# DataCTE/SDXL-Training-Improvements

Measured on AMD Instinct MI355X. Metric: images/sec/node SDXL-base 1024^2 bf16 fwd+bwd, higher is better.
Workload: dtype bf16; 1 GPU; method=ddpm v_prediction + zero_terminal_snr + MinSNR(5), SDXL-base UNet fwd+bwd, batch 4/GPU, 1024^2 (latent 128x128); global_batch=4, parallelism=dp1, weights=synthetic (counter-hash init of the 2,567,463,684-parameter SDXL-base UNet)

## Files before the change

### sdxl-training-improvements_amd/csrc/engine.hip

```cpp
#include "engine.h"

#include <stdarg.h>
#include <stdlib.h>

#ifdef SDXL_DIAG
int g_knobs[SDXL_NKNOBS] = {0};
#endif
static thread_local char g_err[1024] = "";
void sdxl_set_error(const char* fmt, ...) {
  va_list ap;
  va_start(ap, fmt);
  vsnprintf(g_err, sizeof(g_err), fmt, ap);
  va_end(ap);
}
const char* sdxl_get_error() { return g_err; }

#define CHK(x)            \
  do {                    \
    int _r = (x);         \
    if (_r) return _r;    \
  } while (0)

static inline size_t align_up(size_t v, size_t a) { return (v + a - 1) / a * a; }

// ... 44 lines not shown
    if (hipEventCreateWithFlags(&e, hipEventDisableTiming | hipEventDisableSystemFence) != hipSuccess) return nullptr;
    ev_pool.push_back(e);
  }
  return ev_pool[ev_used++];
}
template <class F>
static int on_side(Plan& p, hipStream_t main, F&& fn) {
  Engine& e = *p.eng;
  if (!e.use_side || !e.side || gemm_profiling()) return fn(main);
  hipEvent_t ev = e.next_event();
  if (!ev) { sdxl_set_error("hipEventCreate failed"); return 2; }
  HIP_CHECK_RET(hipEventRecord(ev, main));
  HIP_CHECK_RET(hipStreamWaitEvent(e.side, ev, 0));
  e.side_dirty = true;
  if (!e.side_leaves.empty()) {
    std::vector<std::function<int(hipStream_t)>> v;
    v.swap(e.side_leaves);
    for (auto& leaf : v) CHK(leaf(e.side));
  }
  return fn(e.side);
}
template <class F>
static int side_leaf(Plan& p, hipStream_t main, F&& fn) {
  Engine& e = *p.eng;
  if (!e.use_side || !e.side || gemm_profiling() || KNOB(2) == 16) return on_side(p, main, fn);
  e.side_leaves.emplace_back(std::function<int(hipStream_t)>(fn));
  return 0;
}
static int launch_wgrad_bucket(Plan& p, hipStream_t main, std::vector<GemmP>& v) {
  if (v.empty()) return 0;
  GemmP g = v[0];
  if (v.size() > 1) {
    g.splitk = 1;
    gemm_fill_group(g, v.data(), (int)v.size());
  }
  v.clear();
  if (g.splitk > 1) g.anyorder = 0;
  return on_side(p, main, [&g](hipStream_t s2) -> int { return launch_gemm(g, s2); });
}
int Engine::defer_wgrad(Plan& p, hipStream_t main, const GemmP& g, int grp) {
  for (auto& b : wg_pending) {
    if (b.empty() || (b[0].M == g.M && b[0].N == g.N && b[0].K == g.K && b[0].accumulate == g.accumulate)) {
      b.push_back(g);
      if ((int)b.size() >= grp) return launch_wgrad_bucket(p, main, b);
      return 0;
    }
  }
  wg_pending.emplace_back(1, g);
  if (grp <= 1) return launch_wgrad_bucket(p, main, wg_pending.back());
  return 0;
}
int Engine::flush_wgrads(Plan& p, hipStream_t main) {
  if (!side_leaves.empty()) CHK(on_side(p, main, [](hipStream_t) -> int { return 0; }));
  for (auto& b : wg_pending) CHK(launch_wgrad_bucket(p, main, b));
  return 0;
}
int Engine::flush_ln_params(Plan& p, hipStream_t main) {
  size_t i = 0;
  while (i < ln_pending.size()) {
    LnRedBatch b;
    b.n = 0;
    while (i < ln_pending.size() && b.n < LN_RED_MAX) b.e[b.n++] = ln_pending[i++];
    CHK(on_side(p, main, [&b](hipStream_t s2) -> int { return launch_ln_param_reduce(b, s2); }));
  }
  ln_pending.clear();
  return 0;
// ... 97 lines not shown
  size_t dy32_off = NONE;
  size_t dy_off = NONE;
  Plan::GradDst dx, dres;
  int ggroup = 64;
  Act* gact = nullptr;
  Act* gu = nullptr;
  LinearOp(Act* x_, Act* y_, PRef w_, PRef b_, int K_, int N_, Act* resid_) : x(x_), y(y_), resid(resid_), w(w_), b(b_), K(K_), N(N_) {}
  void describe(const Plan&, sdxl_plan_op_desc* d) const override {
    d->kind = SDXL_OP_LINEAR;
    desc_tensor(d, 0, x); desc_tensor(d, 1, y); desc_tensor(d, 2, resid); desc_tensor(d, 3, gact); desc_tensor(d, 4, gu);
    desc_param(d, w, b);
    d->K = K; d->N = N; d->splitk = splitk; d->wgroup = wgroup; d->crcfg = crcfg; d->crsplit = crsplit; d->fsplit = fsplit; d->dsplit = dsplit;
    d->delta_on = delta_on ? 1 : 0; d->ln_mode = ln_mode; d->ggroup = ggroup; d->resid_alias = resid_alias;
    d->dy_off = dy_off; d->dy32_off = dy32_off; d->dx_out = dx.out; d->dx_addend = dx.addend; d->dres_out = dres.out; d->dres_addend = dres.addend;
    if (ln_mode == 1) desc_lost(d, INTACT_GRAD, 0);
  }
  int fwd(Plan& p, hipStream_t st) override {
    GemmP g = linear_fwd_problem(p.P(x), x->ld(), p.eng->Wp(w), p.P(y), y->ld(), (int)x->rows, N, K, b.off == NONE ? nullptr : p.eng->Wp(b),
                                 resid ? p.P(resid) : nullptr, resid ? resid->ld() : 0);
    if (gact) gemm_attach_geglu_fwd(g, ggroup, p.P(gact), gact->ld());
    if (fsplit > 1 && !hoist_fwd) { g.splitk = fsplit; g.slab = p.F(p.slab_main_off); }
    return launch_gemm(g, st);
  }
  void plan_bwd(Plan& p) override {
    dy_off = y->goff;
    if (resid) {
      resid_alias = p.grad_alias(resid, y) ? 1 : 0;
      if (!resid_alias) dres = p.grad_dst(resid);
    }
    if (gu) dx = p.grad_dst(gu);
    else if (x->need_grad) dx = p.grad_dst(x);
    splitk = linear_wgrad_splitk(N, K, x->rows);
    wgroup = gemm_pick_group(N, K, 1, x->rows, splitk);
    want_slab(p, N, K, 1, splitk);
    crcfg = cr256_wgrad_cfg(N, K, x->rows, b.off != NONE);
    if (crcfg) { crsplit = cr256_pick_splitk(N, K, x->rows, crcfg); want_slab(p, N, K, 1, crsplit); }
    if (!gact) { fsplit = gemm_pick_splitk_small((int)x->rows, N, K, 3); want_slab_main(p, (int)x->rows, N, fsplit); }
    if (const Engine::LoraOpSel* lo = p.eng->lora_op(w)) {
      const size_t tu = lora_grad_tu_elems((int)lo->host.size(), p.eng->lora.rank, (int)x->rows);
      const size_t pf = (size_t)lora_grad_chunks((int)x->rows) * lo->part_unit;
      if (tu > p.lg_tu_elems) p.lg_tu_elems = tu;
      if (pf > p.lg_part_floats) p.lg_part_floats = pf;
    }
    if (delta_attn && !(!gu && x->need_grad)) attn_set_delta_fused(delta_attn, false);
    if (!gu && x->need_grad) {
      dsplit = gemm_pick_splitk_small((int)x->rows, K, N, 2);
      if (KNOB(3) > 1 && N >= (KNOB(4) > 0 ? KNOB(4) : 8192) && N % (64 * KNOB(3)) == 0 && dsplit == 1) dsplit = KNOB(3);
      want_slab_main(p, (int)x->rows, K, dsplit);
      if (delta_attn) {
        delta_on = attn_delta_wanted(delta_attn) && dsplit <= 1 && K % 128 == 0;
        attn_set_delta_fused(delta_attn, delta_on);
      }
      if (SDXL_LN_EPILOGUE && ln_src && KNOB(26) != 0 && dsplit == 1 && dx.addend == NONE && !x->parent && gemm_ln_cfg((int)x->rows, K, N) &&
          ln_fuse_plan(ln_src, p, KNOB(26) == 2 ? 2 : 1))
        ln_mode = KNOB(26) == 2 ? 2 : 1;
    }
  }
  int bwd(Plan& p, hipStream_t st, bool first) override {
    const bf16* dy = p.GP(dy_off);
    const int M = (int)x->rows;
    if (dy32_off != NONE) {
      auto& cs = p.eng->cs_pending;
      for (size_t i = 0; i < cs.size();) {
        LnRedBatch rb;
        rb.n = 0;
        while (i < cs.size() && rb.n < LN_RED_MAX) rb.e[rb.n++] = cs[i++];
// ... 1088 lines not shown
```

### sdxl-training-improvements_amd/csrc/gemm.hip

```cpp
#include "gemm_tiles.h"

#include <stdio.h>
#include <stdlib.h>

#include <type_traits>
#include <vector>

#define BM 128
#ifndef GEMM_DIRECT_EPILOGUE
#define GEMM_DIRECT_EPILOGUE 1
#endif

static int g_mode256 = 1;
static int g_force_cfg = 0;
#ifdef SDXL_DIAG
static int g_sk_mode = 0;
#endif

static constexpr int cdiv_c(int a, int b) { return (a + b - 1) / b; }
__device__ unsigned g_ln_spin_error = 0;
__device__ __forceinline__ float row16_sum(float v) {
  v += __builtin_bit_cast(float, __builtin_amdgcn_update_dpp(0, __builtin_bit_cast(int, v), 0x111, 0xf, 0xf, true));
  v += __builtin_bit_cast(float, __builtin_amdgcn_update_dpp(0, __builtin_bit_cast(int, v), 0x112, 0xf, 0xf, true));
  v += __builtin_bit_cast(float, __builtin_amdgcn_update_dpp(0, __builtin_bit_cast(int, v), 0x114, 0xf, 0xf, true));
// ... 972 lines not shown
          for (int e = 0; e < 8; ++e) {
            oa[e] = (bf16)xa[e];
            ot[e] = (bf16)xt[e];
            og[e] = (bf16)((float)oa[e] * gelu_f((float)ot[e]));
          }
          *(bf16x8*)((bf16*)p.C + (long)m * p.ldc + na) = oa;
          *(bf16x8*)((bf16*)p.C + (long)m * p.ldc + nt) = ot;
          *(bf16x8*)(p.aux + (long)m * p.ldaux + (n0 >> 1) + col) = og;
        } else {
          const int n = n0 + col;
          if (n >= p.N) continue;
          const int Gp = p.geglu_group;
          const long cu = (long)(n / Gp) * (2 * Gp) + (n % Gp);
          bf16x8 ua = *(const bf16x8*)(p.aux + (long)m * p.ldaux + cu);
          bf16x8 ut = *(const bf16x8*)(p.aux + (long)m * p.ldaux + cu + Gp);
          bf16x8 oa, ot;
#pragma unroll
          for (int e = 0; e < 8; ++e) {
            const float dv = (float)(bf16)Cs[row * LDC + col + e], tv = (float)ut[e];
            float cdf, pdf;
            gelu_cdf_pdf(tv, &cdf, &pdf);
            oa[e] = (bf16)(dv * tv * cdf);
            ot[e] = (bf16)(dv * (float)ua[e] * fmaf(tv, pdf, cdf));
          }
          *(bf16x8*)((bf16*)p.C + (long)m * p.ldc + cu) = oa;
          *(bf16x8*)((bf16*)p.C + (long)m * p.ldc + cu + Gp) = ot;
        }
      }
    }
    __syncthreads();
  }
}

__global__ void splitk_reduce_kernel(const float* __restrict__ slab, float* __restrict__ C, int M, int cols, long ldc,
                                     long slab_ld, int splitk, int accumulate, bf16* __restrict__ Cb, float cb_scale,
                                     float* __restrict__ bias_grad) {
  const int vpr = cols / 4;
  for (long i = (long)blockIdx.x * blockDim.x + threadIdx.x; i < (long)M * vpr; i += (long)gridDim.x * blockDim.x) {
    long m = i / vpr;
    int c = (int)(i - m * vpr) * 4;
    if (bias_grad && c == 0) {
      const float* tail = slab + (long)splitk * M * slab_ld + m;
      float b = 0.f;
      for (int s = 0; s < splitk; ++s) b += tail[(long)s * M];
      bias_grad[m] += b;
    }
    f32x4 a = accumulate ? *(const f32x4*)(C + m * ldc + c) : (f32x4){0.f, 0.f, 0.f, 0.f};
    for (int s = 0; s < splitk; ++s) {
      f32x4 v = *(const f32x4*)(slab + ((long)s * M + m) * slab_ld + c);
      a[0] += v[0]; a[1] += v[1]; a[2] += v[2]; a[3] += v[3];
    }
    if (Cb) {
      bf16x4 o;
      o[0] = (bf16)(a[0] * cb_scale); o[1] = (bf16)(a[1] * cb_scale); o[2] = (bf16)(a[2] * cb_scale); o[3] = (bf16)(a[3] * cb_scale);
      *(bf16x4*)(Cb + m * ldc + c) = o;
    } else {
      *(f32x4*)(C + m * ldc + c) = a;
    }
  }
}

__global__ void splitk_epilogue_kernel(const float* __restrict__ slab, bf16* __restrict__ C, int M, int N, long ldc, long slab_ld,
                                       int splitk, const bf16* __restrict__ bias, const bf16* __restrict__ resid, long ldr,
                                       const bf16* __restrict__ rowvec, long ldv, int rows_per_batch) {
  const int vpr = N / 8;
  for (long i = (long)blockIdx.x * blockDim.x + threadIdx.x; i < (long)M * vpr; i += (long)gridDim.x * blockDim.x) {
    const long m = i / vpr;
    const int n = (int)(i - m * vpr) * 8;
    float x[8] = {0.f, 0.f, 0.f, 0.f, 0.f, 0.f, 0.f, 0.f};
    for (int s = 0; s < splitk; ++s) {
      const float* sp = slab + ((long)s * M + m) * slab_ld + n;
      const f32x4 a = *(const f32x4*)sp, b = *(const f32x4*)(sp + 4);
      x[0] += a[0]; x[1] += a[1]; x[2] += a[2]; x[3] += a[3]; x[4] += b[0]; x[5] += b[1]; x[6] += b[2]; x[7] += b[3];
    }
    if (bias) {
      const bf16x8 v = *(const bf16x8*)(bias + n);
#pragma unroll
      for (int e = 0; e < 8; ++e) x[e] += (float)v[e];
    }
    if (rowvec) {
      const bf16x8 v = *(const bf16x8*)(rowvec + (m / rows_per_batch) * ldv + n);
#pragma unroll
      for (int e = 0; e < 8; ++e) x[e] += (float)v[e];
    }
    if (resid) {
      const bf16x8 v = *(const bf16x8*)(resid + m * ldr + n);
#pragma unroll
      for (int e = 0; e < 8; ++e) x[e] += (float)v[e];
    }
    bf16x8 o;
#pragma unroll
    for (int e = 0; e < 8; ++e) o[e] = (bf16)x[e];
// ... 368 lines not shown
    ARG_CHECK(((uintptr_t)p.rowvec & 15) == 0 && p.ldv % 8 == 0 && p.rows_per_batch >= 1,
              "gemm: the row vector must be 16-byte aligned, ldv=%ld a multiple of 8, rows_per_batch=%d at least 1", p.ldv, p.rows_per_batch);
  if (p.form == GEMM_TN) {
    ARG_CHECK(p.M % 8 == 0, "gemm TN: M=%d must be a multiple of 8", p.M);
    ARG_CHECK(p.out_f32, "gemm TN: only fp32 output is implemented");
    ARG_CHECK(p.ldc % 4 == 0, "gemm TN: ldc=%ld must be a multiple of 4", p.ldc);
  } else {
    ARG_CHECK(p.K % 8 == 0, "gemm: K=%d must be a multiple of 8", p.K);
    ARG_CHECK(!p.out_f32, "gemm NT/NN: bf16 output");
    if (p.splitk > 1 && (!gemm_fast_ok(p, 64) || p.geglu || p.N % 8 != 0)) p.splitk = 1;
    ARG_CHECK(p.ldc % 8 == 0, "gemm: ldc=%ld must be a multiple of 8", p.ldc);
    if (p.accumulate) { p.resid = (const bf16*)p.C; p.ldr = p.ldc; }
    if (p.geglu) {
      if (p.geglu_group == 0) p.geglu_group = 64;
      ARG_CHECK(p.geglu == 2 ? p.geglu_group % 8 == 0 : (p.geglu_group == 64 || p.geglu_group == 80), "gemm: geglu group %d (forward: 64 or 80)", p.geglu_group);
      const int G = p.geglu_group;
      ARG_CHECK((p.geglu == 1 && p.form == GEMM_NT && p.N % (2 * G) == 0) || (p.geglu == 2 && p.form == GEMM_NN && p.N % G == 0),
                "gemm: geglu mode %d does not fit form %d / N=%d / group %d", p.geglu, p.form, p.N, G);
      ARG_CHECK(p.aux && p.ldaux % 8 == 0 && ((uintptr_t)p.aux & 15) == 0 && p.taps == 1, "gemm: geglu needs an aligned aux matrix");
      ARG_CHECK(!p.resid && !p.rowvec && (p.geglu == 1 || !p.bias), "gemm: geglu epilogue takes no residual / row vector");
    }
  }
  if (p.form == GEMM_TN) {
    ARG_CHECK(!p.geglu, "gemm TN: no geglu epilogue");
    ARG_CHECK(!p.Cb || (((uintptr_t)p.Cb & 7) == 0), "gemm TN: bf16 destination must be 8-byte aligned");
  } else {
    ARG_CHECK(!p.Cb, "gemm: the bf16 gradient destination is a TN (wgrad) option");
  }
  if (p.splitk < 1) p.splitk = 1;
  if (p.delta_out)
    ARG_CHECK(p.form == GEMM_NN && p.splitk == 1 && p.taps == 1 && !p.geglu && p.delta_o && p.delta_nq > 0 && p.delta_heads > 0 && p.delta_ldo % 8 == 0,
              "gemm: the Delta epilogue takes a plain, unsplit NN problem (form %d, splitk %d)", p.form, p.splitk);
  if (p.group > 1) {
    ARG_CHECK(p.form == GEMM_TN && p.taps == 1 && p.splitk == 1 && p.group <= GEMM_MAX_GROUP,
              "gemm: grouped launches are TN, one tap, no split-K, at most %d problems", GEMM_MAX_GROUP);
    for (int i = 0; i < p.group; ++i)
      ARG_CHECK(p.gA[i] && p.gB[i] && p.gC[i] && (((uintptr_t)p.gA[i] | (uintptr_t)p.gB[i] | (uintptr_t)p.gC[i]) & 15) == 0,
                "gemm: grouped operands must be set and 16-byte aligned");
    p.A = p.gA[0]; p.B = p.gB[0]; p.C = p.gC[0]; p.bias_grad = p.gbias_grad[0]; p.Cb = p.gCb[0];
  } else {
    p.group = 0;
  }
  {
    p.xcd_px = 0;
    {
      const int gx = cdiv(p.N, 128), gy = cdiv(p.M, BM);
      double best = 1e30;
      for (int px = 1; px <= 8; px *= 2) {
        const int py = 8 / px;
        if (gx % px || gy % py) continue;
        double cost = (double)p.N / px + (double)p.M / py;
        if (cost < best) { best = cost; p.xcd_px = px; }
      }
    }
  }
  if (p.splitk > 1) {
    ARG_CHECK(p.slab != nullptr, "gemm: split-K needs a slab scratch buffer");
    if (p.form != GEMM_TN && p.splitk > p.K / 64 * p.taps) p.splitk = p.K / 64 * p.taps;
    p.slab_ld = p.form == GEMM_TN ? (long)p.N * p.taps : (long)p.N;
  }
  if (p.ln_x) {
    ARG_CHECK(SDXL_LN_EPILOGUE, "gemm: the LayerNorm-backward epilogue exists in the diagnostics build only");
    ARG_CHECK(p.form == GEMM_NN && p.taps == 1 && p.splitk == 1 && !p.geglu && !p.resid && !p.bias && !p.rowvec && !p.delta_out && !p.up2,
              "gemm: the LayerNorm-backward epilogue takes a plain NN problem");
    const int lc = gemm_ln_cfg(p.M, p.N, p.K);
    ARG_CHECK(lc != 0 && (p.cfg == lc || p.cfg == 0), "gemm: LayerNorm-backward epilogue: M=%d N=%d K=%d cfg=%d does not fit (gemm_ln_cfg)", p.M, p.N, p.K, p.cfg);
    p.cfg = lc;
    ARG_CHECK(p.ln_stats && p.ln_gamma && p.ln_dx && p.ln_part && p.ln_epoch > 0 && p.ln_ldx % 8 == 0 && p.ln_ldo % 8 == 0 && ((uintptr_t)p.ln_part & 15) == 0 &&
              (((uintptr_t)p.ln_x | (uintptr_t)p.ln_dx | (uintptr_t)p.ln_addend | (uintptr_t)p.ln_gamma) & 15) == 0,
              "gemm: LayerNorm-backward epilogue: missing or misaligned buffers");
  }
  return 0;
}

GemmRoute gemm_route(const GemmP& p) {
  const bool tn = p.form == GEMM_TN, split = p.splitk > 1;
  const int fc = p.cfg > 0 ? p.cfg : g_force_cfg;
  const int post = !split ? GEMM_POST_NONE : tn ? GEMM_POST_REDUCE : GEMM_POST_EPILOGUE;
  auto k128 = [&]() -> GemmRoute {
    const int c = gemm_route_cfg128(p);
    const bool fast = gemm_fast_ok(p, c == 2 ? 32 : 64);
    return {GEMM_K128, c == 23 && !fast ? 3 : c, fast, post};
  };
  if (p.ln_x) return k128();
  {
    bool use = fc == 7 || fc == 8;
    const bool pl_pf = fc == 8 || KNOB(31) == 1;
    if (!use && fc == 0 && KNOB(30) != 64 && p.taps == 1 && !tn) {
      const int bnp = p.N % 160 == 0 ? 160 : 128;
      const long tiles = (long)cdiv(p.M, BM) * cdiv(p.N, bnp);
      const int k30 = KNOB(30) ? KNOB(30) : 3;
      const bool one_round = tiles <= 256 && tiles > 128;
      use = ((k30 & 1) && p.form == GEMM_NT && one_round) || ((k30 & 2) && p.form == GEMM_NN && one_round) || ((k30 & 512) && p.form == GEMM_NN && one_round && p.K >= 2560) ||
            ((k30 & 16) && tiles > 128 && tiles % 256 == 0) || ((k30 & 1024) && p.form == GEMM_NT && tiles > 256 && tiles % 256 == 0) || (k30 & 32);
    }
    if (use && pl_applicable(p)) return {GEMM_KPL, pl_pf ? 8 : 7, false, GEMM_POST_NONE};
  }
  if (fc >= 31 && fc <= 36 && !p.delta_out && cr256_applicable(p)) {
    bool biasg = tn && p.bias_grad;
    for (int i = 0; tn && i < p.group; ++i) biasg = biasg || p.gbias_grad[i];
    return {GEMM_KCR256, fc == 31 && biasg ? 32 : fc, false, tn ? post : GEMM_POST_NONE};
  }
#ifdef SDXL_DIAG
  if (g_sk_mode && !p.delta_out && !(!tn && split) && (g_sk_mode == 2 ? gemm_sk_applicable(p) : gemm_use_sk(p))) return {GEMM_KSK, 0, false, GEMM_POST_NONE};
#endif
  if (g_mode256 && p.group <= 1 && !p.Cb && !p.delta_out && !(!tn && split) && gemm256_applicable(p)) {
    const bool geglu256 = p.geglu == 1 && p.geglu_group == 64 && (long)(p.M / 256) * (p.N / 256) >= 256;
    if (g_mode256 == 2 || gemm_use256(p.form, p.M, p.N, p.K, p.splitk) || geglu256) return {GEMM_K256, 0, false, post};
  }
  if (tn && p.taps != 1 && conv_wgrad3_applicable(p) && conv_wgrad3_policy(p.M, p.N, p.K, p.Wm, p.sm)) return {GEMM_KCONV_WGRAD3, 0, false, post};
  if (tn && p.taps == 1 && wgrad256_applicable(p) && wgrad256_policy(p.M, p.N, p.K)) return {GEMM_KWGRAD256, 0, false, post};
  return k128();
}
int gemm_route_checked(GemmP p, GemmRoute* r) {
  if (int e = gemm_check(p)) return e;
  *r = gemm_route(p);
  return 0;
}

static int launch_gemm_post(const GemmP& p, int post, hipStream_t st) {
  if (post == GEMM_POST_NONE) return 0;
  const int cols = post == GEMM_POST_REDUCE ? p.N * p.taps : p.N;
  const long nv = (long)p.M * (cols / (post == GEMM_POST_REDUCE ? 4 : 8));
  int g = (int)((nv + 255) / 256);
  if (g > 2048) g = 2048;
  if (post == GEMM_POST_REDUCE)
    hipLaunchKernelGGL(splitk_reduce_kernel, dim3(g), dim3(256), 0, st, p.slab, (float*)p.C, p.M, cols, p.ldc, p.slab_ld, p.splitk, p.accumulate, p.Cb,
                       p.cb_scale, p.up2 == 1 ? nullptr : p.bias_grad);
  else
    hipLaunchKernelGGL(splitk_epilogue_kernel, dim3(g), dim3(256), 0, st, p.slab, (bf16*)p.C, p.M, p.N, p.ldc, p.slab_ld, p.splitk,
                       p.bias, p.resid, p.ldr, p.rowvec, p.ldv, p.rows_per_batch > 0 ? p.rows_per_batch : 1);
  HIP_CHECK_RET(hipGetLastError());
  return 0;
}

static int launch_gemm_impl(const GemmP& pin, hipStream_t st) {
  GemmP p = pin;
  if (int e = gemm_check(p)) return e;
  const GemmRoute r = gemm_route(p);
  const bool conv = p.taps != 1;
  int rc;
  switch (r.kernel) {
    case GEMM_KPL: return launch_pl(p, 0, st, r.cfg == 8);
    case GEMM_KCR256: rc = launch_cr256(p, (r.cfg == 31 || r.cfg == 33 || r.cfg == 36) ? 160 : 128, st, r.cfg == 33 || r.cfg == 34, r.cfg == 35 || r.cfg == 36); break;
#ifdef SDXL_DIAG
    case GEMM_KSK: {
      GemmP q = p;
      q.splitk = 1;
      return launch_gemm_sk(&q, 1, st);
    }
#endif
    case GEMM_K256: rc = launch_gemm256(p, st); break;
    case GEMM_KCONV_WGRAD3: rc = launch_conv_wgrad3(p, st); break;
    case GEMM_KWGRAD256: rc = launch_wgrad256(p, st); break;
    default:
      if (p.form == GEMM_NT) rc = conv ? launch_one<GEMM_NT, true>(p, r, st) : launch_one<GEMM_NT, false>(p, r, st);
      else if (p.form == GEMM_TN) rc = conv ? launch_one<GEMM_TN, true>(p, r, st) : launch_one<GEMM_TN, false>(p, r, st);
      else if (p.form == GEMM_NN) rc = conv ? launch_one<GEMM_NN, true>(p, r, st) : launch_one<GEMM_NN, false>(p, r, st);
      else ARG_CHECK(false, "gemm: unknown form %d", p.form);
// ... 123 lines not shown
```

### sdxl-training-improvements_amd/csrc/hooks.hip

```cpp
#include "capi.h"

static int hook_scratch(size_t bytes, void** out) {
  static char* buf = nullptr;
  static size_t cap = 0;
  if (bytes > cap) {
    if (buf) { (void)hipFree(buf); buf = nullptr; cap = 0; }
    HIP_CHECK_RET(hipMalloc((void**)&buf, bytes));
    cap = bytes;
  }
  *out = buf;
  return 0;
}
static int hook_floats(size_t n, float** out) { return hook_scratch(n * sizeof(float), (void**)out); }
static int dense_problem(int form, const void* A, const void* B, void* C, int M, int N, int K, const void* bias, const void* resid, int accumulate,
                         GemmP* g) {
  const bf16 *a = (const bf16*)A, *b = (const bf16*)B, *r = (const bf16*)resid;
  ARG_CHECK(form == GEMM_NT || form == GEMM_NN || form == GEMM_TN, "gemm: unknown form %d", form);
  if (form == GEMM_NT) *g = linear_fwd_problem(a, K, b, C, N, M, N, K, (const bf16*)bias, r, N);
  else if (form == GEMM_NN) { *g = linear_dgrad_problem(a, K, b, C, N, M, N, K, r, N); g->bias = (const bf16*)bias; }
  else { *g = linear_wgrad_problem(a, M, b, N, (float*)C, M, N, K, (float*)bias); if (r) { g->resid = r; g->ldr = N; } }
  g->accumulate = accumulate;
  return 0;
}

// ... 180 lines not shown
  memset(out, 0, sizeof(*out));
  size_t* const offs[] = {&out->dy_off, &out->dx_out, &out->dx_addend, &out->dres_out, &out->dres_addend, &out->d3_out, &out->d3_addend, &out->dy32_off,
                          &out->w_off, &out->b_off, &out->stats_off, &out->lse_off, &out->delta_off, &out->rv32_off, &out->planar_off, &out->weff_off,
                          &out->dweff_off, &out->s2_planar_off};
  for (size_t* o : offs) *o = SDXL_PLAN_NONE;
  for (int r = 0; r < SDXL_PLAN_ROLES; ++r) plan_describe_tensor(out->t[r], nullptr);
  out->intact_after_step = ~0u;
  const Op& op = *p.ops[i];
  out->seg = op.seg; out->hoist_fwd = op.hoist_fwd ? 1 : 0;
  op.describe(p, out);
  return 0;
}
int sdxl_debug_plan_tail(sdxl_handle* h, sdxl_plan_tail* out, size_t out_bytes) {
  ARG_CHECK(out_bytes == sizeof(sdxl_plan_tail), "plan tail: the caller's struct has %zu bytes, the library's %zu", out_bytes, sizeof(sdxl_plan_tail));
  H_CHECK(h);
  ARG_CHECK(h->e.cur, "no plan: call sdxl_plan first");
  ARG_CHECK(out, "null output");
  const Plan& p = *h->e.cur;
  memset(out, 0, sizeof(*out));
  out->B = p.B; out->H = p.H; out->W = p.W; out->ctx = p.ctx;
  plan_describe_tensor(out->x_in, p.x_in); plan_describe_tensor(out->pred, p.pred); plan_describe_tensor(out->ehs, p.ehs);
  out->tp32_off = p.tp32_off; out->tp32_bytes = p.tp32_bytes; out->t_off = p.t_off; out->tid_off = p.tid_off; out->loss_off = p.loss_off;
  out->workspace_bytes = p.ws_bytes;
  return 0;
}

int sdxl_op_wgrad_group(int n, const void* const* dy, const void* const* x, float* const* dw, float* const* dbias, int Mo, int No,
                        int rows, int accumulate, void* st) {
  ARG_CHECK(n >= 1 && n <= GEMM_MAX_GROUP, "wgrad group of %d (1..%d)", n, GEMM_MAX_GROUP);
  GemmP v[GEMM_MAX_GROUP];
  for (int i = 0; i < n; ++i) v[i] = linear_wgrad_problem((const bf16*)dy[i], Mo, (const bf16*)x[i], No, dw[i], Mo, No, rows, dbias ? dbias[i] : nullptr);
  GemmP g = v[0];
  g.accumulate = accumulate;
  gemm_fill_group(g, v, n);
  return launch_gemm(g, (hipStream_t)st);
}

int sdxl_op_conv3x3_fwd(const void* x, const void* w, const void* bias, void* y, int B, int H, int W, int Cin, int Cout,
                        int stride, void* st) {
  GemmP g = conv3x3_fwd_problem(B, H, W, Cin, Cout, stride);
  g.A = (const bf16*)x; g.B = (const bf16*)w; g.C = y;
  g.bias = (const bf16*)bias;
  g.splitk = conv3x3_fwd_splitk(B, H, W, Cin, Cout, stride);
  if (g.splitk > 1) CHK(hook_floats(gemm_slab_floats(g.M, Cout, 1, g.splitk), &g.slab));
  return launch_gemm(g, (hipStream_t)st);
}
int sdxl_op_upconv3x3_fwd(const void* x, const void* w, const void* bias, void* weff, void* planar, void* y, int B, int H, int W,
                          int Cin, int Cout, void* st) {
  const int Mp = 4 * (int)upconv_plane_rows(B, H, W);
  int splitk = upconv3x3_fwd_splitk(B, H, W, Cin, Cout);
  float* slab = nullptr;
  if (splitk > 1) CHK(hook_floats(gemm_slab_floats(Mp, Cout, 1, splitk), &slab));
  return launch_upconv3x3_fwd((const bf16*)x, (const bf16*)w, (const bf16*)bias, (bf16*)weff, (bf16*)planar, (bf16*)y, B, H, W, Cin, Cout,
                              splitk, slab, (hipStream_t)st);
}
int sdxl_op_upconv3x3_dgrad(const void* dy, const void* weff, void* planar, void* dx, const void* addend, int B, int H, int W, int Cin,
                            int Cout, void* st) {
  int splitk = upconv3x3_dgrad_splitk(B, H, W, Cin, Cout);
  float* slab = nullptr;
  if (splitk > 1) CHK(hook_floats(gemm_slab_floats(B * H * W, Cin, 1, splitk), &slab));
  return launch_upconv3x3_dgrad((const bf16*)dy, (const bf16*)weff, (bf16*)planar, (bf16*)dx, (const bf16*)addend, B, H, W, Cin, Cout, splitk,
                                slab, 0, (hipStream_t)st);
}
#ifdef SDXL_DIAG
int sdxl_op_conv3x3_s2_fwd(const void* x, const void* w, const void* bias, void* xplanar, void* y, int B, int H, int W, int Cin, int Cout,
                           void* st) {
// ... 367 lines not shown
```

### sdxl-training-improvements_amd/csrc/kernels.h

```cpp
#pragma once
#include "common.h"

#define SDXL_NKNOBS 40
#ifdef SDXL_DIAG
extern int g_knobs[SDXL_NKNOBS];
#define KNOB(i) (g_knobs[(i)])
constexpr bool SDXL_DIAG_BUILD = true;
constexpr bool SDXL_UP2_3 = true;
constexpr bool SDXL_LN_EPILOGUE = true;
#else
#define KNOB(i) 0
constexpr bool SDXL_DIAG_BUILD = false;
constexpr bool SDXL_UP2_3 = false;
constexpr bool SDXL_LN_EPILOGUE = false;
#endif

enum { GEMM_NT = 0, GEMM_NN = 1, GEMM_TN = 2 };
#define GEMM_LAUNCH(kernel, grid, block, smem, st, p)                                                          \
  do {                                                                                                         \
    if ((p).anyorder) hipExtLaunchKernelGGL(kernel, grid, block, smem, st, nullptr, nullptr, hipExtAnyOrderLaunch, p); \
    else hipLaunchKernelGGL(kernel, grid, block, smem, st, p);                                                 \
  } while (0)

#define GEMM_MAX_GROUP 4
// ... 89 lines not shown
GemmP conv3x3_fwd_problem(int B, int H, int W, int Cin, int Cout, int stride);
GemmP conv3x3_dgrad_problem(int B, int H, int W, int Cin, int Cout, int stride);
GemmP conv3x3_wgrad_problem(int B, int H, int W, int Cin, int Cout, int stride);
GemmP linear_fwd_problem(const bf16* x, long ldx, const bf16* w, void* y, long ldy, int M, int N, int K, const bf16* bias, const bf16* resid, long ldr);
GemmP linear_dgrad_problem(const bf16* dy, long ldy, const bf16* w, void* dx, long ldx, int M, int N, int K, const bf16* addend, long ldr);
GemmP linear_wgrad_problem(const bf16* dy, long ldy, const bf16* x, long ldx, float* dw, int Mo, int No, int rows, float* bias_grad);
void gemm_attach_geglu_fwd(GemmP& g, int group, bf16* gact, long ldgact);
void gemm_attach_geglu_bwd(GemmP& g, int group, bf16* u, long ldu);
void gemm_attach_delta(GemmP& g, const bf16* o, long ldo, float* delta, int nq, int heads);
void gemm_attach_ln_bwd(GemmP& g, const bf16* x, long ldx, const float* stats, const bf16* gamma, bf16* dx, const bf16* addend, float* part, int epoch,
                        float* pcol);
void gemm_fill_group(GemmP& g, const GemmP* v, int n);
int launch_gemm256(const GemmP& p, hipStream_t st);
void gemm256_set_tail(bool on);
#ifdef SDXL_DIAG
bool gemm_sk_applicable(const GemmP& p);
int launch_gemm_sk(const GemmP* problems, int n, hipStream_t st);
int launch_gemm_multi(const GemmP* problems, int n, hipStream_t st);
void gemm_set_sk_mode(int mode);
int gemm_sk_mode();
bool gemm_use_sk(const GemmP& p);
void gemm_sk_set_workers(int n);
int gemm_ln_error(unsigned* out);
int gemm_sk_error(hipStream_t st, unsigned* out);
#endif
bool conv_wgrad3_applicable(const GemmP& p);
bool conv_wgrad3_policy(int M, int N, long red, int Wm, int stride);
int conv_wgrad3_pick_splitk(int M, int N, long red);
int launch_conv_wgrad3(const GemmP& p, hipStream_t st);
void conv_wgrad3_set_enabled(bool on);
bool wgrad256_applicable(const GemmP& p);
bool wgrad256_policy(int M, int N, long red);
int wgrad256_pick_splitk(int M, int N, long red);
int launch_wgrad256(const GemmP& p, hipStream_t st);
void wgrad256_set_enabled(bool on);
bool cr256_applicable(const GemmP& p);
int launch_cr256(const GemmP& p, int bn, hipStream_t st, bool deep = false, bool phased = false);
int cr256_wgrad_cfg(int M, int N, long red, bool bias);
bool pl_applicable(const GemmP& p);
int launch_pl(const GemmP& p, int bn, hipStream_t st, bool prefetch = false);
int launch_pl_prefetch_b(const GemmP& p, int parts, hipStream_t st);
int gemm_ln_cfg(int M, int N, int K);
size_t gemm_ln_part_floats(int M, int N);
size_t gemm_ln_pcol_floats(int M, int N);
int gemm_ln_rowblocks(int M);
int cr256_pick_splitk(int M, int N, long red, int cfg);
int gemm_profile_begin();
FILE* launch_log();
bool gemm_profiling();
int gemm_profile_end(double* flops, double* ms, int* launches);

struct AttnP {
  const bf16 *Q, *K, *V;
  bf16* O;
  float* LSE;
  int B, H, Nq, Nk;
  long ldq, ldk, ldv, ldo;
  const bf16* dO;
  long lddo;
  bf16 *dQ, *dK, *dV;
  long lddq, lddk, lddv;
  float* Delta;
  int accumulate;
  int qsplit;
  float* part;
  int prio;
// ... 320 lines not shown
```

### sdxl-training-improvements_amd/csrc/wgrad256.hip

```cpp
#include "gemm_tiles.h"

namespace {

constexpr int WL_BM = 256, WL_BN = 160, WL_BK = 64, WL_S = 3;
constexpr int WL_A_BYTES = WL_BK * WL_BM * 2;
constexpr int WL_B_BYTES = WL_BK * WL_BN * 2;
constexpr int WL_STAGE = WL_A_BYTES + WL_B_BYTES;
constexpr int WL_SMEM = WL_S * WL_STAGE + 1024;
constexpr int WL_NL = 7;

__global__ __launch_bounds__(512, 2) void wgrad256_kernel(const GemmP p) {
  extern __shared__ __attribute__((aligned(16))) char smem[];
  const int tid = threadIdx.x, lane = tid & 63;
  const int wave = __builtin_amdgcn_readfirstlane(tid >> 6);
  const int wm = wave >> 1, wn = wave & 1;
  const int l16 = lane & 15, g = lane >> 4;
  int bx, by, split;
  xcd_seq_map(p.xcd_bh, bx, by, split);
  const int n0 = bx * WL_BN, m0 = by * WL_BM;
  const int ktiles = p.K / WL_BK;
  const int chunk = (ktiles + p.splitk - 1) / p.splitk;
  const int kt_begin = split * chunk;
  const int kt_end = min(ktiles, kt_begin + chunk);
  const int T = kt_end - kt_begin;
  const bf16* zsrc = (const bf16*)g_zero16;
  const unsigned lds_base = lds_addr_of(smem);
  const unsigned pad_dst = lds_base + WL_S * WL_STAGE;

  const bf16* pa[4];
  long sa[4];
#pragma unroll
  for (int j = 0; j < 4; ++j) {
    const int c = wave + 8 * j;
    const int sub = c >> 4, cc = c & 15;
    const int krow = cc * 4 + (lane >> 4);
    const int m = m0 + sub * 128 + (nc_logical<128>(krow, lane & 15) << 3);
    const bool ok = m < p.M;
    pa[j] = ok ? p.A + ((long)kt_begin * WL_BK + krow) * p.lda + m : zsrc;
    sa[j] = ok ? (long)WL_BK * p.lda : 0;
  }
  const bf16* pb[3];
  long sb[3];
#pragma unroll
  for (int j = 0; j < 3; ++j) {
    const int c = wave + 8 * j;
    const int q = c * 64 + lane;
    const int krow = q / 20, pv = q - krow * 20;
    const int n = n0 + (nc_logical<160>(krow, pv) << 3);
    const bool ok = c < 20 && n < p.N;
    pb[j] = ok ? p.B + ((long)kt_begin * WL_BK + krow) * p.ldb + n : zsrc;
    sb[j] = ok ? (long)WL_BK * p.ldb : 0;
  }
  auto issue_piece = [&](int pc, int slot, bool live) {
    const unsigned At = lds_base + slot * WL_STAGE, Bt = At + WL_A_BYTES;
#pragma unroll
    for (int j = 0; j < 4; ++j)
      if (pc == j) {
        lds_dma16_global(live ? (const void*)pa[j] : (const void*)zsrc, At + (wave + 8 * j) * 1024);
        pa[j] += sa[j];
      }
#pragma unroll
    for (int j = 0; j < 3; ++j)
      if (pc == 4 + j) {
        const int c = wave + 8 * j;
        lds_dma16_global(live ? (const void*)pb[j] : (const void*)zsrc, c < 20 ? Bt + c * 1024 : pad_dst);
        pb[j] += sb[j];
      }
  };
  auto stage = [&](int slot, bool live) {
#pragma unroll
    for (int pc = 0; pc < WL_NL; ++pc) issue_piece(pc, slot, live);
  };

  f32x4 acc[4][5];
#pragma unroll
  for (int i = 0; i < 4; ++i)
#pragma unroll
    for (int j = 0; j < 5; ++j) acc[i][j] = (f32x4){0.f, 0.f, 0.f, 0.f};
  const bool do_bias = p.bias_grad != nullptr && bx == 0 && wn == 0;
  f32x4 accb[4];
#pragma unroll
  for (int i = 0; i < 4; ++i) accb[i] = (f32x4){0.f, 0.f, 0.f, 0.f};
  bf16x8 ones;
#pragma unroll
  for (int e = 0; e < 8; ++e) ones[e] = (bf16)1.0f;

  stage(0, 0 < T);
  stage(1, 1 < T);
  int rd = 0, wr = 2;
  for (int t = 0; t < T; ++t) {
    wait_vmcnt<WL_NL>();
    __builtin_amdgcn_s_barrier();
    const bool live = t + 2 < T;
    const char* At = smem + rd * WL_STAGE + (wm >> 1) * (WL_A_BYTES / 2);
    const char* Bt = smem + rd * WL_STAGE + WL_A_BYTES;
    int pc = 0;
#pragma unroll
    for (int ks = 0; ks < 2; ++ks) {
      bf16x8 fa[4], fb[5];
#pragma unroll
      for (int i = 0; i < 4; ++i) fa[i] = frag_nc<128>(At, ks * 32 + g * 8, (wm & 1) * 64 + i * 16, l16);
#pragma unroll
      for (int j = 0; j < 5; ++j) fb[j] = frag_nc<160>(Bt, ks * 32 + g * 8, wn * 80 + j * 16, l16);
      if (do_bias) {
#pragma unroll
        for (int i = 0; i < 4; ++i) accb[i] = __builtin_amdgcn_mfma_f32_16x16x32_bf16(fa[i], ones, accb[i], 0, 0, 0);
      }
#pragma unroll
      for (int i = 0; i < 4; ++i) {
#pragma unroll
        for (int j = 0; j < 5; ++j)
          acc[i][j] = __builtin_amdgcn_mfma_f32_16x16x32_bf16(fb[j], fa[i], acc[i][j], 0, 0, 0);
        if (pc < WL_NL) { issue_piece(pc, wr, live); }
        ++pc;
      }
    }
    rd = rd + 1 == WL_S ? 0 : rd + 1;
    wr = wr + 1 == WL_S ? 0 : wr + 1;
  }
  wait_vmcnt<0>();

  if (do_bias && l16 == 0) {
#pragma unroll
    for (int i = 0; i < 4; ++i)
#pragma unroll
      for (int r = 0; r < 4; ++r) {
        const int m = m0 + wm * 64 + i * 16 + g * 4 + r;
        if (m < p.M) gemm_bias_out(p.bias_grad, p.slab, p.slab_ld, p.splitk, split, p.M, m, accb[i][r]);
      }
  }
#pragma unroll
  for (int i = 0; i < 4; ++i) {
    const int m = m0 + wm * 64 + i * 16 + l16;
    if (m >= p.M) continue;
#pragma unroll
    for (int j = 0; j < 5; ++j) {
      const int n = n0 + wn * 80 + j * 16 + g * 4;
      if (n >= p.N) continue;
      f32x4 x = acc[i][j];
      float* c = (float*)p.C + (long)m * p.ldc + n;
      if (p.splitk > 1) {
        *(f32x4*)(p.slab + ((long)split * p.M + m) * p.slab_ld + n) = x;
      } else if (p.Cb) {
        if (p.accumulate) {
          const f32x4 a = *(const f32x4*)c;
          x[0] += a[0]; x[1] += a[1]; x[2] += a[2]; x[3] += a[3];
        }
        bf16x4 o;
        o[0] = (bf16)(x[0] * p.cb_scale); o[1] = (bf16)(x[1] * p.cb_scale);
        o[2] = (bf16)(x[2] * p.cb_scale); o[3] = (bf16)(x[3] * p.cb_scale);
        *(bf16x4*)(p.Cb + (long)m * p.ldc + n) = o;
      } else if (p.accumulate) {
        f32x4 a = *(f32x4*)c;
        a[0] += x[0]; a[1] += x[1]; a[2] += x[2]; a[3] += x[3];
        *(f32x4*)c = a;
      } else {
        *(f32x4*)c = x;
      }
    }
  }
}

bool g_wl_enabled = true;

}

void wgrad256_set_enabled(bool on) { g_wl_enabled = on; }

bool wgrad256_policy(int M, int N, long red) {
  return g_wl_enabled && red >= 16384 && red % WL_BK == 0 && M % 8 == 0 && N % 8 == 0;
}
bool wgrad256_applicable(const GemmP& p) {
  if (p.form != GEMM_TN || p.taps != 1 || p.group > 1 || !p.out_f32) return false;
  if (p.K % WL_BK || p.M % 8 || p.N % 8 || p.lda % 8 || p.ldb % 8 || p.ldc % 4) return false;
  return true;
}
int wgrad256_pick_splitk(int M, int N, long red) {
  const long tiles = (long)cdiv(M, WL_BM) * cdiv(N, WL_BN);
  const long ktiles = red / WL_BK;
  const long target = KNOB(13) > 0 ? KNOB(13) : 144;
  long s = (target + tiles / 2) / tiles;
  if (s < 1) s = 1;
  while (s > 1 && ktiles / s < 16) --s;
  if (s > 32) s = 32;
  return (int)s;
}

int launch_wgrad256(const GemmP& p, hipStream_t st) {
  ARG_CHECK(wgrad256_applicable(p), "wgrad256: problem does not fit (TN, one tap, K %% 64 == 0)");
  static bool attr_set = false;
  if (!attr_set) {
    HIP_CHECK_RET(hipFuncSetAttribute((const void*)wgrad256_kernel, hipFuncAttributeMaxDynamicSharedMemorySize, WL_SMEM));
    attr_set = true;
  }
  dim3 grid(cdiv(p.N, WL_BN), cdiv(p.M, WL_BM), p.splitk);
  GemmP q = p;
  q.xcd_bh = KNOB(34) == 1 ? 0 : xcd_band_rows(grid.x, grid.y, grid.z, WL_BM, WL_BN);
  GEMM_LAUNCH(wgrad256_kernel, grid, dim3(512), WL_SMEM, st, q);
  HIP_CHECK_RET(hipGetLastError());
  return 0;
}
```

Before: 36.73 images/sec.

## Group small long-reduction weight-gradient GEMMs into one split-K wgrad256 launch

```diff
diff --git a/sdxl-training-improvements_amd/csrc/engine.hip b/sdxl-training-improvements_amd/csrc/engine.hip
--- a/sdxl-training-improvements_amd/csrc/engine.hip
+++ b/sdxl-training-improvements_amd/csrc/engine.hip
@@ -100,6 +100,7 @@
   GemmP g = v[0];
   if (v.size() > 1) {
     g.splitk = 1;
+    wgrad256_group_policy(g.M, g.N, g.K, (int)v.size(), &g.splitk);
     gemm_fill_group(g, v.data(), (int)v.size());
   }
   v.clear();
@@ -263,6 +264,7 @@
     else if (x->need_grad) dx = p.grad_dst(x);
     splitk = linear_wgrad_splitk(N, K, x->rows);
     wgroup = gemm_pick_group(N, K, 1, x->rows, splitk);
+    if (wgroup <= 1) wgroup = wgrad256_group_policy(N, K, x->rows, 0, nullptr);
     want_slab(p, N, K, 1, splitk);
     crcfg = cr256_wgrad_cfg(N, K, x->rows, b.off != NONE);
     if (crcfg) { crsplit = cr256_pick_splitk(N, K, x->rows, crcfg); want_slab(p, N, K, 1, crsplit); }
diff --git a/sdxl-training-improvements_amd/csrc/gemm.hip b/sdxl-training-improvements_amd/csrc/gemm.hip
--- a/sdxl-training-improvements_amd/csrc/gemm.hip
+++ b/sdxl-training-improvements_amd/csrc/gemm.hip
@@ -1028,9 +1028,9 @@
   }
 }
 
-__global__ void splitk_reduce_kernel(const float* __restrict__ slab, float* __restrict__ C, int M, int cols, long ldc,
-                                     long slab_ld, int splitk, int accumulate, bf16* __restrict__ Cb, float cb_scale,
-                                     float* __restrict__ bias_grad) {
+__device__ __forceinline__ void splitk_reduce_body(const float* __restrict__ slab, float* __restrict__ C, int M, int cols, long ldc,
+                                                   long slab_ld, int splitk, int accumulate, bf16* __restrict__ Cb, float cb_scale,
+                                                   float* __restrict__ bias_grad) {
   const int vpr = cols / 4;
   for (long i = (long)blockIdx.x * blockDim.x + threadIdx.x; i < (long)M * vpr; i += (long)gridDim.x * blockDim.x) {
     long m = i / vpr;
@@ -1054,6 +1054,21 @@
       *(f32x4*)(C + m * ldc + c) = a;
     }
   }
+}
+__global__ void splitk_reduce_kernel(const float* __restrict__ slab, float* __restrict__ C, int M, int cols, long ldc,
+                                     long slab_ld, int splitk, int accumulate, bf16* __restrict__ Cb, float cb_scale,
+                                     float* __restrict__ bias_grad) {
+  splitk_reduce_body(slab, C, M, cols, ldc, slab_ld, splitk, accumulate, Cb, cb_scale, bias_grad);
+}
+struct SplitkReduceGroup {
+  float* C[GEMM_MAX_GROUP];
+  bf16* Cb[GEMM_MAX_GROUP];
+  float* bias_grad[GEMM_MAX_GROUP];
+};
+__global__ void splitk_reduce_group_kernel(const float* __restrict__ slab, const SplitkReduceGroup g, int M, int cols, long ldc, long slab_ld,
+                                           int splitk, int accumulate, float cb_scale) {
+  const int i = blockIdx.z;
+  splitk_reduce_body(slab + (long)i * splitk * M * (slab_ld + 1), g.C[i], M, cols, ldc, slab_ld, splitk, accumulate, g.Cb[i], cb_scale, g.bias_grad[i]);
 }
 
 __global__ void splitk_epilogue_kernel(const float* __restrict__ slab, bf16* __restrict__ C, int M, int N, long ldc, long slab_ld,
@@ -1488,8 +1503,8 @@
     ARG_CHECK(p.form == GEMM_NN && p.splitk == 1 && p.taps == 1 && !p.geglu && p.delta_o && p.delta_nq > 0 && p.delta_heads > 0 && p.delta_ldo % 8 == 0,
               "gemm: the Delta epilogue takes a plain, unsplit NN problem (form %d, splitk %d)", p.form, p.splitk);
   if (p.group > 1) {
-    ARG_CHECK(p.form == GEMM_TN && p.taps == 1 && p.splitk == 1 && p.group <= GEMM_MAX_GROUP,
-              "gemm: grouped launches are TN, one tap, no split-K, at most %d problems", GEMM_MAX_GROUP);
+    ARG_CHECK(p.form == GEMM_TN && p.taps == 1 && p.group <= GEMM_MAX_GROUP && (p.splitk == 1 || (wgrad256_applicable(p) && wgrad256_policy(p.M, p.N, p.K))),
+              "gemm: grouped launches are TN, one tap, no split-K (but on the long-reduction kernel), at most %d problems", GEMM_MAX_GROUP);
     for (int i = 0; i < p.group; ++i)
       ARG_CHECK(p.gA[i] && p.gB[i] && p.gC[i] && (((uintptr_t)p.gA[i] | (uintptr_t)p.gB[i] | (uintptr_t)p.gC[i]) & 15) == 0,
                 "gemm: grouped operands must be set and 16-byte aligned");
@@ -1539,6 +1554,7 @@
     return {GEMM_K128, c == 23 && !fast ? 3 : c, fast, post};
   };
   if (p.ln_x) return k128();
+  if (tn && p.group > 1 && split) return {GEMM_KWGRAD256, 0, false, GEMM_POST_REDUCE};
   {
     bool use = fc == 7 || fc == 8;
     const bool pl_pf = fc == 8 || KNOB(31) == 1;
@@ -1565,7 +1581,7 @@
     if (g_mode256 == 2 || gemm_use256(p.form, p.M, p.N, p.K, p.splitk) || geglu256) return {GEMM_K256, 0, false, post};
   }
   if (tn && p.taps != 1 && conv_wgrad3_applicable(p) && conv_wgrad3_policy(p.M, p.N, p.K, p.Wm, p.sm)) return {GEMM_KCONV_WGRAD3, 0, false, post};
-  if (tn && p.taps == 1 && wgrad256_applicable(p) && wgrad256_policy(p.M, p.N, p.K)) return {GEMM_KWGRAD256, 0, false, post};
+  if (tn && p.taps == 1 && p.group <= 1 && wgrad256_applicable(p) && wgrad256_policy(p.M, p.N, p.K)) return {GEMM_KWGRAD256, 0, false, post};
   return k128();
 }
 int gemm_route_checked(GemmP p, GemmRoute* r) {
@@ -1580,7 +1596,13 @@
   const long nv = (long)p.M * (cols / (post == GEMM_POST_REDUCE ? 4 : 8));
   int g = (int)((nv + 255) / 256);
   if (g > 2048) g = 2048;
-  if (post == GEMM_POST_REDUCE)
+  if (post == GEMM_POST_REDUCE && p.group > 1) {
+    SplitkReduceGroup rg;
+    memset(&rg, 0, sizeof(rg));
+    for (int i = 0; i < p.group; ++i) { rg.C[i] = p.gC[i]; rg.Cb[i] = p.gCb[i]; rg.bias_grad[i] = p.gbias_grad[i]; }
+    hipLaunchKernelGGL(splitk_reduce_group_kernel, dim3(g, 1, p.group), dim3(256), 0, st, p.slab, rg, p.M, cols, p.ldc, p.slab_ld, p.splitk, p.accumulate,
+                       p.cb_scale);
+  } else if (post == GEMM_POST_REDUCE)
     hipLaunchKernelGGL(splitk_reduce_kernel, dim3(g), dim3(256), 0, st, p.slab, (float*)p.C, p.M, cols, p.ldc, p.slab_ld, p.splitk, p.accumulate, p.Cb,
                        p.cb_scale, p.up2 == 1 ? nullptr : p.bias_grad);
   else
diff --git a/sdxl-training-improvements_amd/csrc/hooks.hip b/sdxl-training-improvements_amd/csrc/hooks.hip
--- a/sdxl-training-improvements_amd/csrc/hooks.hip
+++ b/sdxl-training-improvements_amd/csrc/hooks.hip
@@ -236,6 +236,8 @@
   for (int i = 0; i < n; ++i) v[i] = linear_wgrad_problem((const bf16*)dy[i], Mo, (const bf16*)x[i], No, dw[i], Mo, No, rows, dbias ? dbias[i] : nullptr);
   GemmP g = v[0];
   g.accumulate = accumulate;
+  wgrad256_group_policy(Mo, No, rows, n, &g.splitk);
+  if (g.splitk > 1) CHK(hook_floats((size_t)n * gemm_slab_floats(Mo, No, 1, g.splitk), &g.slab));
   gemm_fill_group(g, v, n);
   return launch_gemm(g, (hipStream_t)st);
 }
diff --git a/sdxl-training-improvements_amd/csrc/kernels.h b/sdxl-training-improvements_amd/csrc/kernels.h
--- a/sdxl-training-improvements_amd/csrc/kernels.h
+++ b/sdxl-training-improvements_amd/csrc/kernels.h
@@ -145,6 +145,7 @@
 bool wgrad256_applicable(const GemmP& p);
 bool wgrad256_policy(int M, int N, long red);
 int wgrad256_pick_splitk(int M, int N, long red);
+int wgrad256_group_policy(int M, int N, long red, int n, int* splitk);
 int launch_wgrad256(const GemmP& p, hipStream_t st);
 void wgrad256_set_enabled(bool on);
 bool cr256_applicable(const GemmP& p);
diff --git a/sdxl-training-improvements_amd/csrc/wgrad256.hip b/sdxl-training-improvements_amd/csrc/wgrad256.hip
--- a/sdxl-training-improvements_amd/csrc/wgrad256.hip
+++ b/sdxl-training-improvements_amd/csrc/wgrad256.hip
@@ -17,6 +17,15 @@
   const int l16 = lane & 15, g = lane >> 4;
   int bx, by, split;
   xcd_seq_map(p.xcd_bh, bx, by, split);
+  const bf16 *gA = p.A, *gB = p.B;
+  float *gC = (float*)p.C, *gbias = p.bias_grad, *gslab = p.slab;
+  bf16* gCb = p.Cb;
+  if (p.group > 1) {
+    const int prob = split / p.splitk;
+    split -= prob * p.splitk;
+    gA = p.gA[prob]; gB = p.gB[prob]; gC = p.gC[prob]; gbias = p.gbias_grad[prob]; gCb = p.gCb[prob];
+    if (p.splitk > 1) gslab += (long)prob * p.splitk * p.M * (p.slab_ld + 1);
+  }
   const int n0 = bx * WL_BN, m0 = by * WL_BM;
   const int ktiles = p.K / WL_BK;
   const int chunk = (ktiles + p.splitk - 1) / p.splitk;
@@ -36,7 +45,7 @@
     const int krow = cc * 4 + (lane >> 4);
     const int m = m0 + sub * 128 + (nc_logical<128>(krow, lane & 15) << 3);
     const bool ok = m < p.M;
-    pa[j] = ok ? p.A + ((long)kt_begin * WL_BK + krow) * p.lda + m : zsrc;
+    pa[j] = ok ? gA + ((long)kt_begin * WL_BK + krow) * p.lda + m : zsrc;
     sa[j] = ok ? (long)WL_BK * p.lda : 0;
   }
   const bf16* pb[3];
@@ -48,7 +57,7 @@
     const int krow = q / 20, pv = q - krow * 20;
     const int n = n0 + (nc_logical<160>(krow, pv) << 3);
     const bool ok = c < 20 && n < p.N;
-    pb[j] = ok ? p.B + ((long)kt_begin * WL_BK + krow) * p.ldb + n : zsrc;
+    pb[j] = ok ? gB + ((long)kt_begin * WL_BK + krow) * p.ldb + n : zsrc;
     sb[j] = ok ? (long)WL_BK * p.ldb : 0;
   }
   auto issue_piece = [&](int pc, int slot, bool live) {
@@ -77,7 +86,7 @@
   for (int i = 0; i < 4; ++i)
 #pragma unroll
     for (int j = 0; j < 5; ++j) acc[i][j] = (f32x4){0.f, 0.f, 0.f, 0.f};
-  const bool do_bias = p.bias_grad != nullptr && bx == 0 && wn == 0;
+  const bool do_bias = gbias != nullptr && bx == 0 && wn == 0;
   f32x4 accb[4];
 #pragma unroll
   for (int i = 0; i < 4; ++i) accb[i] = (f32x4){0.f, 0.f, 0.f, 0.f};
@@ -126,7 +135,7 @@
 #pragma unroll
       for (int r = 0; r < 4; ++r) {
         const int m = m0 + wm * 64 + i * 16 + g * 4 + r;
-        if (m < p.M) gemm_bias_out(p.bias_grad, p.slab, p.slab_ld, p.splitk, split, p.M, m, accb[i][r]);
+        if (m < p.M) gemm_bias_out(gbias, gslab, p.slab_ld, p.splitk, split, p.M, m, accb[i][r]);
       }
   }
 #pragma unroll
@@ -138,10 +147,10 @@
       const int n = n0 + wn * 80 + j * 16 + g * 4;
       if (n >= p.N) continue;
       f32x4 x = acc[i][j];
-      float* c = (float*)p.C + (long)m * p.ldc + n;
+      float* c = gC + (long)m * p.ldc + n;
       if (p.splitk > 1) {
-        *(f32x4*)(p.slab + ((long)split * p.M + m) * p.slab_ld + n) = x;
-      } else if (p.Cb) {
+        *(f32x4*)(gslab + ((long)split * p.M + m) * p.slab_ld + n) = x;
+      } else if (gCb) {
         if (p.accumulate) {
           const f32x4 a = *(const f32x4*)c;
           x[0] += a[0]; x[1] += a[1]; x[2] += a[2]; x[3] += a[3];
@@ -149,7 +158,7 @@
         bf16x4 o;
         o[0] = (bf16)(x[0] * p.cb_scale); o[1] = (bf16)(x[1] * p.cb_scale);
         o[2] = (bf16)(x[2] * p.cb_scale); o[3] = (bf16)(x[3] * p.cb_scale);
-        *(bf16x4*)(p.Cb + (long)m * p.ldc + n) = o;
+        *(bf16x4*)(gCb + (long)m * p.ldc + n) = o;
       } else if (p.accumulate) {
         f32x4 a = *(f32x4*)c;
         a[0] += x[0]; a[1] += x[1]; a[2] += x[2]; a[3] += x[3];
@@ -171,7 +180,7 @@
   return g_wl_enabled && red >= 16384 && red % WL_BK == 0 && M % 8 == 0 && N % 8 == 0;
 }
 bool wgrad256_applicable(const GemmP& p) {
-  if (p.form != GEMM_TN || p.taps != 1 || p.group > 1 || !p.out_f32) return false;
+  if (p.form != GEMM_TN || p.taps != 1 || p.group > GEMM_MAX_GROUP || !p.out_f32) return false;
   if (p.K % WL_BK || p.M % 8 || p.N % 8 || p.lda % 8 || p.ldb % 8 || p.ldc % 4) return false;
   return true;
 }
@@ -185,6 +194,29 @@
   if (s > 32) s = 32;
   return (int)s;
 }
+#ifndef WL_GROUP
+#define WL_GROUP 2
+#endif
+int wgrad256_group_policy(int M, int N, long red, int n, int* splitk) {
+  if (splitk) *splitk = 1;
+  const long tiles = (long)cdiv(M, WL_BM) * cdiv(N, WL_BN);
+  if (!wgrad256_policy(M, N, red) || tiles > 16 || WL_GROUP < 2) return 1;
+  const int grp = WL_GROUP > GEMM_MAX_GROUP ? GEMM_MAX_GROUP : WL_GROUP;
+  if (n <= 0) n = grp;
+  if (n > GEMM_MAX_GROUP) n = GEMM_MAX_GROUP;
+  const long alone = wgrad256_pick_splitk(M, N, red);
+  if (red / WL_BK / alone >= 32) return 1;
+  long s = alone;
+  if (n > 1) {
+    const long target = KNOB(13) > 0 ? KNOB(13) : 144;
+    s = (target + n * tiles / 2) / (n * tiles);
+    while (s > 1 && red / WL_BK / s < 32) --s;
+    if (s > alone / n) s = alone / n;
+    if (s < 1) s = 1;
+  }
+  if (splitk) *splitk = (int)s;
+  return grp;
+}
 
 int launch_wgrad256(const GemmP& p, hipStream_t st) {
   ARG_CHECK(wgrad256_applicable(p), "wgrad256: problem does not fit (TN, one tap, K %% 64 == 0)");
@@ -193,7 +225,7 @@
     HIP_CHECK_RET(hipFuncSetAttribute((const void*)wgrad256_kernel, hipFuncAttributeMaxDynamicSharedMemorySize, WL_SMEM));
     attr_set = true;
   }
-  dim3 grid(cdiv(p.N, WL_BN), cdiv(p.M, WL_BM), p.splitk);
+  dim3 grid(cdiv(p.N, WL_BN), cdiv(p.M, WL_BM), (p.group > 1 ? p.group : 1) * p.splitk);
   GemmP q = p;
   q.xcd_bh = KNOB(34) == 1 ? 0 : xcd_band_rows(grid.x, grid.y, grid.z, WL_BM, WL_BN);
   GEMM_LAUNCH(wgrad256_kernel, grid, dim3(512), WL_SMEM, st, q);
```

After: 36.52 images/sec. About the same (-0.6%).
